# luo-yining/CFDBench

Measured on NVIDIA H100. Metric: fno_rollout_steps_per_sec, higher is better.
Workload: dtype bf16

## Files before the change

cfdbench_b200/csrc/fno_project_tc.cu:

```cuda
#include "fno_common.cuh"
#include "tc_common.cuh"

namespace fno {

constexpr int kPtWG = 4;
constexpr int kPtThreads = 128 * kPtWG;
constexpr int kPtM = kW;
constexpr uint32_t kPtLboA = (kPtM / 8) * 128;
constexpr uint32_t kPtLboB = (kProj / 8) * 128;
constexpr int kPtTilesPerSample = kH;
constexpr int kPtReps = kPtM * (kC / 4) / 128;

struct PtSmem {
  alignas(128) float w_hi[kProj * kC];
  alignas(128) float w_lo[kProj * kC];
  alignas(128) float a_hi[kPtWG][kPtM * kC];
  alignas(128) float a_lo[kPtWG][kPtM * kC];
  alignas(16) float4 w2q[kProj / 2];
  alignas(16) float2 b1p[kProj / 2];
};

template <typename TAct>
struct PtRegs {
  TAct v[kPtReps][4];
};

template <typename TAct>
__device__ __forceinline__ void pt_prefetch(PtRegs<TAct>& r, const TAct* __restrict__ a, int tile, int t) {
  const int b = tile / kPtTilesPerSample, p0 = (tile % kPtTilesPerSample) * kPtM;
#pragma unroll
  for (int rep = 0; rep < kPtReps; ++rep) {
    const int task = rep * 128 + t;
    const int m = task & (kPtM - 1), kq = task >> 6;
    const TAct* src = a + (static_cast<size_t>(b) * kC + 4 * kq) * kHW + p0 + m;
#pragma unroll
    for (int c = 0; c < 4; ++c) r.v[rep][c] = __ldg(src + static_cast<size_t>(c) * kHW);
  }
}

__device__ __forceinline__ float pt_to_float(float v) { return v; }
__device__ __forceinline__ float pt_to_float(__nv_bfloat16 v) { return __bfloat162float(v); }

template <typename TAct>
__device__ __forceinline__ void pt_split_store(const PtRegs<TAct>& r, float* a_hi, float* a_lo, int t) {
#pragma unroll
  for (int rep = 0; rep < kPtReps; ++rep) {
    const int task = rep * 128 + t;
    const int m = task & (kPtM - 1), kq = task >> 6;
    float hi[4], lo[4];
#pragma unroll
    for (int c = 0; c < 4; ++c) {
      const float x = pt_to_float(r.v[rep][c]);
      if constexpr (sizeof(TAct) == 4) tc::split_tf32(x, hi[c], lo[c]);
      else hi[c] = x;
    }
    const uint32_t off = tc::kmajor_offset(m, 4 * kq, kPtM) / 4;
    *reinterpret_cast<float4*>(a_hi + off) = make_float4(hi[0], hi[1], hi[2], hi[3]);
    if constexpr (sizeof(TAct) == 4) *reinterpret_cast<float4*>(a_lo + off) = make_float4(lo[0], lo[1], lo[2], lo[3]);
  }
}

template <typename TAct>
__global__ void __launch_bounds__(kPtThreads, 1)
    project_tc_kernel(const TAct* __restrict__ a, const float* __restrict__ w1, const float* __restrict__ b1,
                      const float* __restrict__ w2, const float* __restrict__ b2, const float* __restrict__ mask,
                      float* __restrict__ preds, int n_tiles) {
  constexpr bool kBf16 = sizeof(TAct) == 2;
  extern __shared__ __align__(1024) unsigned char smem_raw[];
  PtSmem& sm = *reinterpret_cast<PtSmem*>(smem_raw);
  const int tid = threadIdx.x, lane = tid & 31;
  const int wg = tc::warp_index_uniform() >> 2, t = tid & 127, wq = (tid >> 5) & 3;

  for (int e = tid; e < kProj * kC; e += kPtThreads) {
    const int j = e / kC, i = e % kC;
    float hi, lo;
    tc::split_tf32(w1[e], hi, lo);
    const uint32_t off = tc::kmajor_offset(j, i, kProj) / 4;
    sm.w_hi[off] = hi;
    sm.w_lo[off] = lo;
  }
  if (tid < kProj / 2) {
    sm.w2q[tid] = make_float4(w2[2 * tid], w2[kProj + 2 * tid], w2[2 * tid + 1], w2[kProj + 2 * tid + 1]);
    sm.b1p[tid] = make_float2(b1[2 * tid], b1[2 * tid + 1]);
  }
  const float b2x = b2[0], b2y = b2[1];
  tc::fence_proxy_async_smem();
  __syncthreads();
  pdl_wait();
  pdl_launch_dependents();

  const int first = blockIdx.x * kPtWG + wg, stride = gridDim.x * kPtWG;
  float* a_hi = sm.a_hi[wg];
  float* a_lo = sm.a_lo[wg];
  PtRegs<TAct> regs;
  if (first < n_tiles) pt_prefetch<TAct>(regs, a, first, t);
  for (int tile = first; tile < n_tiles; tile += stride) {
    pt_split_store<TAct>(regs, a_hi, a_lo, t);
    tc::fence_proxy_async_smem();
    tc::named_barrier(1 + wg, 128);
    if (tile + stride < n_tiles) pt_prefetch<TAct>(regs, a, tile + stride, t);
    float acc[64];
    tc::wg_fence();
    {
      const uint32_t a_s[3] = {tc::smem_addr(a_hi), tc::smem_addr(a_lo), tc::smem_addr(a_hi)};
      const uint32_t b_s[3] = {tc::smem_addr(sm.w_hi), tc::smem_addr(sm.w_hi), tc::smem_addr(sm.w_lo)};
#pragma unroll
      for (int pass = 0; pass < 3; ++pass) {
        if (kBf16 && pass == 1) continue;
#pragma unroll
        for (int ks = 0; ks < kC / 8; ++ks)
          tc::wg_tf32_ss_n128(acc, tc::make_smem_desc(a_s[pass] + ks * 2 * kPtLboA, kPtLboA, 128),
                              tc::make_smem_desc(b_s[pass] + ks * 2 * kPtLboB, kPtLboB, 128), (pass | ks) ? 1u : 0u);
      }
    }
    tc::wg_commit();
    tc::wg_wait<0>();
    tc::wg_fence_acc(acc);
    const int b = tile / kPtTilesPerSample, p0 = (tile % kPtTilesPerSample) * kPtM;
#pragma unroll
    for (int hh = 0; hh < 2; ++hh) {
      float2 out = make_float2(0.f, 0.f);
#pragma unroll
      for (int i0 = 0; i0 < 16; i0 += 8) {
        float2 g[8];
#pragma unroll
        for (int i = 0; i < 8; ++i) {
          const float2 bb = sm.b1p[4 * (i0 + i) + (lane & 3)];
          g[i] = make_float2(acc[4 * (i0 + i) + 2 * hh] + bb.x, acc[4 * (i0 + i) + 2 * hh + 1] + bb.y);
        }
        if constexpr (kBf16) {
          gelu_erf2_deg5_batch<8>(g);
        } else {
#pragma unroll
          for (int i = 0; i < 8; ++i) g[i] = gelu_erf2(g[i]);
        }
#pragma unroll
        for (int i = 0; i < 8; ++i) {
          const float4 wq4 = sm.w2q[4 * (i0 + i) + (lane & 3)];
          out = ffma2(make_float2(g[i].x, g[i].x), make_float2(wq4.x, wq4.y), out);
          out = ffma2(make_float2(g[i].y, g[i].y), make_float2(wq4.z, wq4.w), out);
        }
      }
      out.x += __shfl_xor_sync(0xffffffffu, out.x, 1);
      out.y += __shfl_xor_sync(0xffffffffu, out.y, 1);
      out.x += __shfl_xor_sync(0xffffffffu, out.x, 2);
      out.y += __shfl_xor_sync(0xffffffffu, out.y, 2);
      if ((lane & 3) == 0) {
        const int pix = p0 + 16 * wq + (lane >> 2) + 8 * hh;
        const float mk = __ldg(mask + static_cast<size_t>(b) * kHW + pix);
        preds[(static_cast<size_t>(b) * 2 + 0) * kHW + pix] = (b2x + out.x) * mk;
        preds[(static_cast<size_t>(b) * 2 + 1) * kHW + pix] = (b2y + out.y) * mk;
      }
    }
  }
}

template <typename TAct>
cudaError_t launch_project_tc(const void* a, const float* w1, const float* b1, const float* w2, const float* b2,
                              const float* mask, float* preds, int batch, cudaStream_t stream) {
  auto kern = project_tc_kernel<TAct>;
  constexpr size_t smem = sizeof(PtSmem);
  static PerDeviceLaunch pd;
  int n_sm = 0;
  cudaError_t e0 = per_device_setup(kern, smem, pd, &n_sm);
  if (e0 != cudaSuccess) return e0;
  const int n_tiles = batch * kPtTilesPerSample;
  const int want = (n_tiles + kPtWG - 1) / kPtWG;
  const int grid = want < n_sm ? want : n_sm;
  return launch_chained(kern, dim3(grid), dim3(kPtThreads), smem, stream, static_cast<const TAct*>(a), w1, b1, w2, b2,
                        mask, preds, n_tiles);
}
template cudaError_t launch_project_tc<float>(const void*, const float*, const float*, const float*, const float*,
                                              const float*, float*, int, cudaStream_t);
template cudaError_t launch_project_tc<__nv_bfloat16>(const void*, const float*, const float*, const float*,
                                                      const float*, const float*, float*, int, cudaStream_t);

}
```

Before: 1353.

## Feed projection kernel via TMA ring buffer and register-A wgmma with split-N overlap

Replaces per-thread global loads and shared-memory split stores of the activation tile with TMA 3D loads into a 4-slot swizzled mbarrier ring per warpgroup. The A operand now comes from registers, via the register-source wgmma variant, instead of an fp32 shared-memory copy. The N=128 GEMM is split into two N=64 halves so the GELU/projection epilogue of one half overlaps the tensor-core work of the other. The aim is to cut load latency and shared-memory traffic in the projection stage, at the cost of added mbarrier, tensor-map setup and register-pressure complexity; the fp32 path drops to 3 warpgroups.

```diff
diff --git a/cfdbench_b200/csrc/fno_project_tc.cu b/cfdbench_b200/csrc/fno_project_tc.cu
--- a/cfdbench_b200/csrc/fno_project_tc.cu
+++ b/cfdbench_b200/csrc/fno_project_tc.cu
@@ -1,77 +1,66 @@
 #include "fno_common.cuh"
 #include "tc_common.cuh"
+#include "tc_tma.cuh"
 
 namespace fno {
 
-constexpr int kPtWG = 4;
-constexpr int kPtThreads = 128 * kPtWG;
-constexpr int kPtM = kW;
-constexpr uint32_t kPtLboA = (kPtM / 8) * 128;
+template <typename TAct>
+constexpr int kPtWG = sizeof(TAct) == 2 ? 4 : 3;
 constexpr uint32_t kPtLboB = (kProj / 8) * 128;
+constexpr uint32_t kPtHalfB = (kProj / 2 / 8) * 128;
 constexpr int kPtTilesPerSample = kH;
-constexpr int kPtReps = kPtM * (kC / 4) / 128;
-
+constexpr int kPtSlots = 4;
+
+__host__ __device__ constexpr int pt_tile(int c, int wg, int n, int grid, int wgs) { return c + (wgs * n + wg) * grid; }
+__host__ __device__ constexpr int pt_slot(int n) { return n % kPtSlots; }
+__host__ __device__ constexpr uint32_t pt_parity(int n) { return static_cast<uint32_t>(n / kPtSlots) & 1u; }
+
+template <typename TAct>
+struct PtRow {
+  static constexpr uint32_t kBoxW = 128 / sizeof(TAct);
+  static constexpr int kBoxes = kW / kBoxW;
+  static constexpr uint32_t kBoxBytes = kBoxW * kC * sizeof(TAct);
+  static constexpr uint32_t kBytes = kBoxes * kBoxBytes;
+  static __device__ __forceinline__ uint32_t offset(int c, int w) {
+    constexpr int kChunk = 16 / sizeof(TAct);
+    const int e = w % kBoxW;
+    return (w / kBoxW) * kBoxBytes + c * 128 + ((((e / kChunk) ^ c) & 7) << 4) + (e % kChunk) * sizeof(TAct);
+  }
+};
+
+template <typename TAct>
 struct PtSmem {
+  alignas(1024) unsigned char x[kPtWG<TAct>][kPtSlots][PtRow<TAct>::kBytes];
   alignas(128) float w_hi[kProj * kC];
   alignas(128) float w_lo[kProj * kC];
-  alignas(128) float a_hi[kPtWG][kPtM * kC];
-  alignas(128) float a_lo[kPtWG][kPtM * kC];
   alignas(16) float4 w2q[kProj / 2];
   alignas(16) float2 b1p[kProj / 2];
+  alignas(8) uint64_t full[kPtWG<TAct>][kPtSlots];
 };
-
-template <typename TAct>
-struct PtRegs {
-  TAct v[kPtReps][4];
-};
-
-template <typename TAct>
-__device__ __forceinline__ void pt_prefetch(PtRegs<TAct>& r, const TAct* __restrict__ a, int tile, int t) {
-  const int b = tile / kPtTilesPerSample, p0 = (tile % kPtTilesPerSample) * kPtM;
-#pragma unroll
-  for (int rep = 0; rep < kPtReps; ++rep) {
-    const int task = rep * 128 + t;
-    const int m = task & (kPtM - 1), kq = task >> 6;
-    const TAct* src = a + (static_cast<size_t>(b) * kC + 4 * kq) * kHW + p0 + m;
-#pragma unroll
-    for (int c = 0; c < 4; ++c) r.v[rep][c] = __ldg(src + static_cast<size_t>(c) * kHW);
-  }
-}
 
 __device__ __forceinline__ float pt_to_float(float v) { return v; }
 __device__ __forceinline__ float pt_to_float(__nv_bfloat16 v) { return __bfloat162float(v); }
 
 template <typename TAct>
-__device__ __forceinline__ void pt_split_store(const PtRegs<TAct>& r, float* a_hi, float* a_lo, int t) {
-#pragma unroll
-  for (int rep = 0; rep < kPtReps; ++rep) {
-    const int task = rep * 128 + t;
-    const int m = task & (kPtM - 1), kq = task >> 6;
-    float hi[4], lo[4];
-#pragma unroll
-    for (int c = 0; c < 4; ++c) {
-      const float x = pt_to_float(r.v[rep][c]);
-      if constexpr (sizeof(TAct) == 4) tc::split_tf32(x, hi[c], lo[c]);
-      else hi[c] = x;
-    }
-    const uint32_t off = tc::kmajor_offset(m, 4 * kq, kPtM) / 4;
-    *reinterpret_cast<float4*>(a_hi + off) = make_float4(hi[0], hi[1], hi[2], hi[3]);
-    if constexpr (sizeof(TAct) == 4) *reinterpret_cast<float4*>(a_lo + off) = make_float4(lo[0], lo[1], lo[2], lo[3]);
-  }
-}
-
-template <typename TAct>
-__global__ void __launch_bounds__(kPtThreads, 1)
-    project_tc_kernel(const TAct* __restrict__ a, const float* __restrict__ w1, const float* __restrict__ b1,
-                      const float* __restrict__ w2, const float* __restrict__ b2, const float* __restrict__ mask,
-                      float* __restrict__ preds, int n_tiles) {
+__global__ void __launch_bounds__(128 * kPtWG<TAct>, 1)
+    project_tc_kernel(const __grid_constant__ CUtensorMap a_map, const float* __restrict__ w1,
+                      const float* __restrict__ b1, const float* __restrict__ w2, const float* __restrict__ b2,
+                      const float* __restrict__ mask, float* __restrict__ preds, int n_tiles) {
   constexpr bool kBf16 = sizeof(TAct) == 2;
+  constexpr int kWG = kPtWG<TAct>;
+  using Row = PtRow<TAct>;
   extern __shared__ __align__(1024) unsigned char smem_raw[];
-  PtSmem& sm = *reinterpret_cast<PtSmem*>(smem_raw);
+  PtSmem<TAct>& sm = *reinterpret_cast<PtSmem<TAct>*>(smem_raw);
+  if ((smem_u32(smem_raw) & 1023u) != 0) __trap();
   const int tid = threadIdx.x, lane = tid & 31;
   const int wg = tc::warp_index_uniform() >> 2, t = tid & 127, wq = (tid >> 5) & 3;
 
-  for (int e = tid; e < kProj * kC; e += kPtThreads) {
+  if (tid == 0) {
+    for (int g = 0; g < kWG; ++g)
+      for (int s = 0; s < kPtSlots; ++s) mbar_init(&sm.full[g][s], 1);
+    fence_mbar_init();
+  }
+  for (int e = tid; e < kProj * kC; e += 128 * kWG) {
     const int j = e / kC, i = e % kC;
     float hi, lo;
     tc::split_tf32(w1[e], hi, lo);
@@ -89,86 +78,148 @@
   pdl_wait();
   pdl_launch_dependents();
 
-  const int first = blockIdx.x * kPtWG + wg, stride = gridDim.x * kPtWG;
-  float* a_hi = sm.a_hi[wg];
-  float* a_lo = sm.a_lo[wg];
-  PtRegs<TAct> regs;
-  if (first < n_tiles) pt_prefetch<TAct>(regs, a, first, t);
-  for (int tile = first; tile < n_tiles; tile += stride) {
-    pt_split_store<TAct>(regs, a_hi, a_lo, t);
-    tc::fence_proxy_async_smem();
-    tc::named_barrier(1 + wg, 128);
-    if (tile + stride < n_tiles) pt_prefetch<TAct>(regs, a, tile + stride, t);
-    float acc[64];
+  const int grid = gridDim.x, tile0 = pt_tile(blockIdx.x, wg, 0, grid, kWG), tstride = kWG * grid;
+  const int n_fills = tile0 < n_tiles ? (n_tiles - tile0 + tstride - 1) / tstride : 0;
+  auto fill = [&](int n) {
+    const int tile = pt_tile(blockIdx.x, wg, n, grid, kWG), s = pt_slot(n);
+    const int b = tile / kPtTilesPerSample, h = tile % kPtTilesPerSample;
+    mbar_expect_tx(&sm.full[wg][s], Row::kBytes);
+#pragma unroll
+    for (int box = 0; box < Row::kBoxes; ++box)
+      tma_load_3d(sm.x[wg][s] + box * Row::kBoxBytes, &a_map, box * Row::kBoxW, h, b * kC, &sm.full[wg][s]);
+  };
+  if (t == 0)
+    for (int n = 0; n < kPtSlots && n < n_fills; ++n) fill(n);
+
+  const int q = lane & 3, m0 = 16 * wq + (lane >> 2);
+  const float4* w2q = sm.w2q;
+  const float2* b1p = sm.b1p;
+  uint32_t fa[kBf16 ? 1 : 2][kC / 8][4];
+  auto load_frags = [&](int n) {
+    const int s = pt_slot(n);
+    mbar_wait(&sm.full[wg][s], pt_parity(n));
+    const unsigned char* slot = sm.x[wg][s];
+#pragma unroll
+    for (int ks = 0; ks < kC / 8; ++ks)
+#pragma unroll
+      for (int j = 0; j < 4; ++j) {
+        const float x =
+            pt_to_float(*reinterpret_cast<const TAct*>(slot + Row::offset(8 * ks + q + 4 * (j >> 1), m0 + 8 * (j & 1))));
+        if constexpr (kBf16) {
+          fa[0][ks][j] = __float_as_uint(x);
+        } else {
+          float hi, lo;
+          tc::split_tf32(x, hi, lo);
+          fa[0][ks][j] = __float_as_uint(hi);
+          fa[kBf16 ? 0 : 1][ks][j] = __float_as_uint(lo);
+        }
+      }
+  };
+  auto issue_half = [&](float (&d)[32], int hf) {
+    const uint32_t b_s[3] = {tc::smem_addr(sm.w_hi), tc::smem_addr(sm.w_hi), tc::smem_addr(sm.w_lo)};
     tc::wg_fence();
-    {
-      const uint32_t a_s[3] = {tc::smem_addr(a_hi), tc::smem_addr(a_lo), tc::smem_addr(a_hi)};
-      const uint32_t b_s[3] = {tc::smem_addr(sm.w_hi), tc::smem_addr(sm.w_hi), tc::smem_addr(sm.w_lo)};
-#pragma unroll
-      for (int pass = 0; pass < 3; ++pass) {
-        if (kBf16 && pass == 1) continue;
-#pragma unroll
-        for (int ks = 0; ks < kC / 8; ++ks)
-          tc::wg_tf32_ss_n128(acc, tc::make_smem_desc(a_s[pass] + ks * 2 * kPtLboA, kPtLboA, 128),
-                              tc::make_smem_desc(b_s[pass] + ks * 2 * kPtLboB, kPtLboB, 128), (pass | ks) ? 1u : 0u);
-      }
+#pragma unroll
+    for (int pass = 0; pass < 3; ++pass) {
+      if (kBf16 && pass == 1) continue;
+#pragma unroll
+      for (int ks = 0; ks < kC / 8; ++ks)
+        tc::wg_tf32_rs_n64(d, fa[kBf16 ? 0 : (pass == 1)][ks],
+                           tc::make_smem_desc(b_s[pass] + hf * kPtHalfB + ks * 2 * kPtLboB, kPtLboB, 128),
+                           (pass | ks) ? 1u : 0u);
     }
     tc::wg_commit();
+  };
+  auto epilogue_half = [&](const float (&d)[32], int hf, float2 (&out)[2]) {
+#pragma unroll
+    for (int hh = 0; hh < 2; ++hh) {
+      const int i0 = 8 * hf;
+      float2 g[8];
+#pragma unroll
+      for (int i = 0; i < 8; ++i) {
+        const float2 bb = b1p[4 * (i0 + i) + q];
+        g[i] = make_float2(d[4 * i + 2 * hh] + bb.x, d[4 * i + 2 * hh + 1] + bb.y);
+      }
+      if constexpr (kBf16) {
+        gelu_erf2_deg5_batch<8>(g);
+      } else {
+#pragma unroll
+        for (int i = 0; i < 8; ++i) g[i] = gelu_erf2(g[i]);
+      }
+#pragma unroll
+      for (int i = 0; i < 8; ++i) {
+        const float4 wq4 = w2q[4 * (i0 + i) + q];
+        out[hh] = ffma2(make_float2(g[i].x, g[i].x), make_float2(wq4.x, wq4.y), out[hh]);
+        out[hh] = ffma2(make_float2(g[i].y, g[i].y), make_float2(wq4.z, wq4.w), out[hh]);
+      }
+    }
+  };
+
+  if (n_fills == 0) return;
+  float acc[2][32];
+  load_frags(0);
+  issue_half(acc[0], 0);
+  for (int n = 0; n < n_fills; ++n) {
+    const int tile = pt_tile(blockIdx.x, wg, n, grid, kWG);
+    const int b = tile / kPtTilesPerSample, p0 = (tile % kPtTilesPerSample) * kW;
+    float mk[2] = {0.f, 0.f};
+    if (q == 0) {
+      mk[0] = __ldg(mask + static_cast<size_t>(b) * kHW + p0 + m0);
+      mk[1] = __ldg(mask + static_cast<size_t>(b) * kHW + p0 + m0 + 8);
+    }
+    issue_half(acc[1], 1);
+    float2 out[2] = {make_float2(0.f, 0.f), make_float2(0.f, 0.f)};
+    tc::wg_wait<1>();
+    tc::wg_fence_acc(acc[0]);
+    if (t == 0 && n + kPtSlots < n_fills) fill(n + kPtSlots);
+    epilogue_half(acc[0], 0, out);
     tc::wg_wait<0>();
-    tc::wg_fence_acc(acc);
-    const int b = tile / kPtTilesPerSample, p0 = (tile % kPtTilesPerSample) * kPtM;
+    tc::wg_fence_acc(acc[1]);
+    if (n + 1 < n_fills) load_frags(n + 1);
+    issue_half(acc[0], 0);
+    epilogue_half(acc[1], 1, out);
 #pragma unroll
     for (int hh = 0; hh < 2; ++hh) {
-      float2 out = make_float2(0.f, 0.f);
-#pragma unroll
-      for (int i0 = 0; i0 < 16; i0 += 8) {
-        float2 g[8];
-#pragma unroll
-        for (int i = 0; i < 8; ++i) {
-          const float2 bb = sm.b1p[4 * (i0 + i) + (lane & 3)];
-          g[i] = make_float2(acc[4 * (i0 + i) + 2 * hh] + bb.x, acc[4 * (i0 + i) + 2 * hh + 1] + bb.y);
-        }
-        if constexpr (kBf16) {
-          gelu_erf2_deg5_batch<8>(g);
-        } else {
-#pragma unroll
-          for (int i = 0; i < 8; ++i) g[i] = gelu_erf2(g[i]);
-        }
-#pragma unroll
-        for (int i = 0; i < 8; ++i) {
-          const float4 wq4 = sm.w2q[4 * (i0 + i) + (lane & 3)];
-          out = ffma2(make_float2(g[i].x, g[i].x), make_float2(wq4.x, wq4.y), out);
-          out = ffma2(make_float2(g[i].y, g[i].y), make_float2(wq4.z, wq4.w), out);
-        }
-      }
-      out.x += __shfl_xor_sync(0xffffffffu, out.x, 1);
-      out.y += __shfl_xor_sync(0xffffffffu, out.y, 1);
-      out.x += __shfl_xor_sync(0xffffffffu, out.x, 2);
-      out.y += __shfl_xor_sync(0xffffffffu, out.y, 2);
-      if ((lane & 3) == 0) {
-        const int pix = p0 + 16 * wq + (lane >> 2) + 8 * hh;
-        const float mk = __ldg(mask + static_cast<size_t>(b) * kHW + pix);
-        preds[(static_cast<size_t>(b) * 2 + 0) * kHW + pix] = (b2x + out.x) * mk;
-        preds[(static_cast<size_t>(b) * 2 + 1) * kHW + pix] = (b2y + out.y) * mk;
-      }
-    }
-  }
+      float2 o = out[hh];
+      o.x += __shfl_xor_sync(0xffffffffu, o.x, 1);
+      o.y += __shfl_xor_sync(0xffffffffu, o.y, 1);
+      o.x += __shfl_xor_sync(0xffffffffu, o.x, 2);
+      o.y += __shfl_xor_sync(0xffffffffu, o.y, 2);
+      if (q == 0) {
+        const int pix = p0 + m0 + 8 * hh;
+        preds[(static_cast<size_t>(b) * 2 + 0) * kHW + pix] = (b2x + o.x) * mk[hh];
+        preds[(static_cast<size_t>(b) * 2 + 1) * kHW + pix] = (b2y + o.y) * mk[hh];
+      }
+    }
+  }
+  tc::wg_wait<0>();
 }
 
 template <typename TAct>
 cudaError_t launch_project_tc(const void* a, const float* w1, const float* b1, const float* w2, const float* b2,
                               const float* mask, float* preds, int batch, cudaStream_t stream) {
   auto kern = project_tc_kernel<TAct>;
-  constexpr size_t smem = sizeof(PtSmem);
+  using Row = PtRow<TAct>;
+  constexpr size_t smem = sizeof(PtSmem<TAct>);
+  static_assert(smem <= 232448, "project_tc_kernel: shared memory over the per-block opt-in limit");
   static PerDeviceLaunch pd;
   int n_sm = 0;
   cudaError_t e0 = per_device_setup(kern, smem, pd, &n_sm);
   if (e0 != cudaSuccess) return e0;
+  if (reinterpret_cast<uintptr_t>(a) & 15) return cudaErrorMisalignedAddress;
+  thread_local struct { const void* a = nullptr; int batch = 0; CUtensorMap map; } last;
+  if (last.a != a || last.batch != batch) {
+    last.a = nullptr;
+    e0 = make_tma_map_3d(&last.map, sizeof(TAct) == 2 ? CU_TENSOR_MAP_DATA_TYPE_BFLOAT16 : CU_TENSOR_MAP_DATA_TYPE_FLOAT32,
+                         sizeof(TAct), a, kW, kH, static_cast<uint64_t>(batch) * kC, Row::kBoxW, 1, kC);
+    if (e0 != cudaSuccess) return e0;
+    last.a = a;
+    last.batch = batch;
+  }
+  const CUtensorMap a_map = last.map;
   const int n_tiles = batch * kPtTilesPerSample;
-  const int want = (n_tiles + kPtWG - 1) / kPtWG;
+  const int want = (n_tiles + kPtWG<TAct> - 1) / kPtWG<TAct>;
   const int grid = want < n_sm ? want : n_sm;
-  return launch_chained(kern, dim3(grid), dim3(kPtThreads), smem, stream, static_cast<const TAct*>(a), w1, b1, w2, b2,
-                        mask, preds, n_tiles);
+  return launch_chained(kern, dim3(grid), dim3(128 * kPtWG<TAct>), smem, stream, a_map, w1, b1, w2, b2, mask, preds, n_tiles);
 }
 template cudaError_t launch_project_tc<float>(const void*, const float*, const float*, const float*, const float*,
                                               const float*, float*, int, cudaStream_t);
```

After: 1366, median of 6. No clear change (+0.9%).
